# CVMI-Lab/DODA

Hardware: AMD Instinct MI355X
Metric: active-voxels/sec fwd+bwd SparseConv U-Net, ScanNet 2cm (higher is better)
Workload: dtype bf16; 1 GPU; cfgs/scannet SparseConv U-Net training step (voxel pooling + fwd + CE + bwd + SGD), 2 cm voxels, 4 scenes/GPU x ~150000 active voxels, random-init weights; global_batch=4, voxels_per_gpu=601279, points_per_gpu=781042, parallelism=dp1, n_classes=20, grad_sync=deferred multi-layer wgrad + bucketed all-reduce, collectives=none (single process), prefetch_gate=off, grad_exchange=no process group

## Files before the change

doda_amd/csrc/spconv_wlds.hip:

```cpp
#include "common.hpp"
#include "spconv_common.hpp"

namespace {

constexpr int WK = 27, WCH = 48, WNB = 3;
constexpr int W_SLOTS = 96;
constexpr int W_LDS_BYTES = WK * WNB * W_SLOTS * 16;

template <int S, bool STATS>
__device__ __forceinline__ void wlds_epilogue(f32x4 (&acc)[S], const u32x2 (&pre_res)[S], const u32x2 (&pre_bnx)[S], int row0,
                                              int i, int g, int wid, int nb, int n_out, __amdgpu_buffer_rsrc_t rs_y,
                                              const void *__restrict__ res, const EpiArgs &ep, int part, f32x4 (*sred)[2][4],
                                              const float (*bnv)[WCH]) {
    const unsigned col = (unsigned)(nb * 16 + 4 * g);
    f32x4 st1 = {0.f, 0.f, 0.f, 0.f}, st2 = {0.f, 0.f, 0.f, 0.f};
    auto unpack = [](const u32x2 &v) {
        return (f32x4){__uint_as_float(v[0] << 16), __uint_as_float(v[0] & 0xffff0000u),
                       __uint_as_float(v[1] << 16), __uint_as_float(v[1] & 0xffff0000u)};
    };
#pragma unroll
    for (int s = 0; s < S; ++s) {
        const unsigned t = (unsigned)(row0 + s * 16 + i);
        const unsigned voff = t < (unsigned)n_out ? (t * (ep.y_ld ? ep.y_ld : (unsigned)WCH) + col) * 2u : OOB;
        f32x4 a = acc[s];
        if (res) a += unpack(pre_res[s]);
        u32x2 packed_out;
        packed_out[0] = (unsigned)f2bf(a[0]) | ((unsigned)f2bf(a[1]) << 16);
        packed_out[1] = (unsigned)f2bf(a[2]) | ((unsigned)f2bf(a[3]) << 16);
        if constexpr (STATS) {
            f32x4 v = unpack(packed_out);
            if (ep.bn_x) {
                const f32x4 xr = unpack(pre_bnx[s]);
                const f32x4 mu = *reinterpret_cast<const f32x4 *>(&bnv[0][col]);
                const f32x4 is = *reinterpret_cast<const f32x4 *>(&bnv[1][col]);
                const f32x4 xh = (xr - mu) * is;
                if (ep.bn_relu) {
                    const f32x4 ga = *reinterpret_cast<const f32x4 *>(&bnv[2][col]);
                    const f32x4 be = *reinterpret_cast<const f32x4 *>(&bnv[3][col]);
                    const f32x4 yv = xh * ga + be;
#pragma unroll
                    for (int q = 0; q < 4; ++q) v[q] = yv[q] > 0.f ? v[q] : 0.f;
                }
                st1 += v;
                st2 += v * xh;
            } else {
                st1 += v;
                st2 += v * v;
            }
        }
        __builtin_amdgcn_raw_buffer_store_b64(packed_out, rs_y, voff, 0, 0);
    }
    if constexpr (STATS) {
#pragma unroll
        for (int q = 0; q < 4; ++q) { st1[q] = row_sum16(st1[q]); st2[q] = row_sum16(st2[q]); }
        if (i == 15) { sred[wid][0][g] = st1; sred[wid][1][g] = st2; }
        doda_sync();
        if (wid == 0 && i == 15) {
            f32x4 a1 = sred[0][0][g], a2 = sred[0][1][g];
#pragma unroll
            for (int w = 1; w < 8; ++w) { a1 += sred[w][0][g]; a2 += sred[w][1][g]; }
            stats_emit(ep, (long long)part, WCH, col, a1, a2);
        }
        doda_sync();
    }
}

template <bool STATS>
__global__ __launch_bounds__(512) void conv_wlds48(const unsigned short *__restrict__ x, unsigned x_bytes,
                                                   const u32x4 *__restrict__ wp, const int32_t *__restrict__ tbl,
                                                   unsigned tbl_bytes, int ld, int n_out, void *__restrict__ y,
                                                   unsigned y_bytes, const void *__restrict__ res, const EpiArgs ep) {
    constexpr int S = 2, RW = 16 * S, TM = 8 * RW;
    extern __shared__ __attribute__((aligned(16))) unsigned char wl_raw[];
    u32x4 *wl = reinterpret_cast<u32x4 *>(wl_raw);
    __shared__ f32x4 sred[STATS ? 8 : 1][2][4];
    __shared__ __attribute__((aligned(16))) float bnv[4][WCH];

    const int tid = threadIdx.x, lane = tid & 63, wid = __builtin_amdgcn_readfirstlane(tid >> 6);
    const int i = lane & 15, g = lane >> 4;
    const __amdgpu_buffer_rsrc_t rs_x = __builtin_amdgcn_make_buffer_rsrc((void *)x, 0, x_bytes, 0x00020000);
    const __amdgpu_buffer_rsrc_t rs_t = __builtin_amdgcn_make_buffer_rsrc((void *)tbl, 0, tbl_bytes, 0x00020000);
    const __amdgpu_buffer_rsrc_t rs_y = __builtin_amdgcn_make_buffer_rsrc((void *)y, 0, y_bytes, 0x00020000);

    if constexpr (STATS) {
        if (ep.bn_x && tid < 4 * WCH) {
            const int v = tid / WCH, c = tid - v * WCH;
            const float *src = v == 0 ? ep.bn_mean : v == 1 ? ep.bn_invstd : v == 2 ? ep.bn_gamma : ep.bn_beta;
            bnv[v][c] = src ? src[c] : 0.f;
        }
    }
    const int n_tiles = (n_out + TM - 1) / TM;
    unsigned off[WK][S];
    auto load_table = [&](int tile) {
        const int row0 = tile * TM + wid * RW;
#pragma unroll
        for (int o = 0; o < WK; ++o)
#pragma unroll
            for (int s = 0; s < S; ++s) {
                const int t = row0 + s * 16 + i;
                const unsigned voff = t < n_out ? ((unsigned)o * (unsigned)ld + (unsigned)t) * 4u : OOB;
                off[o][s] = __builtin_amdgcn_raw_buffer_load_b32(rs_t, voff, 0, 0);
            }
    };
    {
        constexpr int NCP = (WK * WNB * W_SLOTS + 511) / 512;
        u32x4 tmp[NCP];
#pragma unroll
        for (int k = 0; k < NCP; ++k) {
            const int e = k * 512 + tid, ec = e < WK * WNB * W_SLOTS ? e : 0;
            const int slot = ec % W_SLOTS, onb = ec / W_SLOTS, nb = onb % WNB, o = onb / WNB;
            const int src = slot < 64 ? ((o * 2 + 0) * WNB + nb) * 64 + slot : ((o * 2 + 1) * WNB + nb) * 64 + (slot - 64);
            tmp[k] = wp[src];
        }
        load_table((int)blockIdx.x);
#pragma unroll
        for (int k = 0; k < NCP; ++k) {
            const int e = k * 512 + tid;
            if (e < WK * WNB * W_SLOTS) wl[e] = tmp[k];
        }
    }
    doda_sync();

    for (int tile = blockIdx.x; tile < n_tiles; tile += gridDim.x) {
        const int row0 = tile * TM + wid * RW;
        u32x2 pre_res[WNB][S], pre_bnx[WNB][S];
        {
            const unsigned rl = ep.res_ld ? ep.res_ld : (unsigned)WCH, bl = ep.bnx_ld ? ep.bnx_ld : (unsigned)WCH;
            const unsigned dense_bytes = (unsigned)n_out * (unsigned)WCH * 2u;
            const __amdgpu_buffer_rsrc_t rs_r = __builtin_amdgcn_make_buffer_rsrc(
                (void *)res, 0, ep.res_ld ? ((unsigned)(n_out - 1) * rl + (unsigned)WCH) * 2u : dense_bytes, 0x00020000);
            const __amdgpu_buffer_rsrc_t rs_b = __builtin_amdgcn_make_buffer_rsrc(
                (void *)ep.bn_x, 0, ep.bnx_ld ? ((unsigned)(n_out - 1) * bl + (unsigned)WCH) * 2u : dense_bytes, 0x00020000);
#pragma unroll
            for (int nb = 0; nb < WNB; ++nb)
#pragma unroll
                for (int s = 0; s < S; ++s) {
                    const unsigned t = (unsigned)(row0 + s * 16 + i);
                    const unsigned cc = (unsigned)(nb * 16 + 4 * g);
                    const unsigned voff = t < (unsigned)n_out ? (t * rl + cc) * 2u : OOB;
                    const unsigned voff_b = t < (unsigned)n_out ? (t * bl + cc) * 2u : OOB;
                    pre_res[nb][s] = __builtin_amdgcn_raw_buffer_load_b64(rs_r, res ? voff : OOB, 0, 0);
                    if constexpr (STATS) pre_bnx[nb][s] = __builtin_amdgcn_raw_buffer_load_b64(rs_b, ep.bn_x ? voff_b : OOB, 0, 0);
                    else pre_bnx[nb][s] = (u32x2){0u, 0u};
                }
        }
        if (tile != (int)blockIdx.x) load_table(tile);
#pragma unroll
        for (int o = 0; o < WK; ++o)
#pragma unroll
            for (int s = 0; s < S; ++s) {
                const int t = row0 + s * 16 + i;
                off[o][s] = (t < n_out && (int)off[o][s] >= 0) ? off[o][s] * (unsigned)(WCH * 2) : OOB;
            }

        f32x4 acc[WNB][S];
#pragma unroll
        for (int nb = 0; nb < WNB; ++nb)
#pragma unroll
            for (int s = 0; s < S; ++s) acc[nb][s] = (f32x4){0.f, 0.f, 0.f, 0.f};

        auto gather = [&](int u, u32x4 (&xa)[S]) {
            const int o = u >> 1, c = u & 1;
#pragma unroll
            for (int s = 0; s < S; ++s) {
                const unsigned base = off[o][s];
                const unsigned voff = (c == 0 || g < 2) && base != OOB ? base + (unsigned)(c * 64 + g * 16) : OOB;
                xa[s] = __builtin_amdgcn_raw_buffer_load_b128(rs_x, voff, 0, 0);
            }
        };
        constexpr int NUNIT = 2 * WK;
        constexpr int PD = 4;
        u32x4 xa[PD + 1][S];
#pragma unroll
        for (int u = 0; u < PD; ++u) gather(u, xa[u]);
#pragma unroll
        for (int u = 0; u < NUNIT; ++u) {
            if (u + PD < NUNIT) gather(u + PD, xa[(u + PD) % (PD + 1)]);
            const int o = u >> 1, c = u & 1;
            u32x4 wf[WNB];
#pragma unroll
            for (int nb = 0; nb < WNB; ++nb) {
                const u32x4 *frag = wl + (o * WNB + nb) * W_SLOTS;
                wf[nb] = c == 0 ? frag[lane] : (g < 2 ? frag[64 + lane] : (u32x4){0u, 0u, 0u, 0u});
            }
            __builtin_amdgcn_sched_barrier(0);
#pragma unroll
            for (int nb = 0; nb < WNB; ++nb)
#pragma unroll
                for (int s = 0; s < S; ++s) mma_bf16_k32(acc[nb][s], wf[nb], xa[u % (PD + 1)][s]);
            __builtin_amdgcn_sched_barrier(0);
        }
#pragma unroll
        for (int nb = 0; nb < WNB; ++nb)
            wlds_epilogue<S, STATS>(acc[nb], pre_res[nb], pre_bnx[nb], row0, i, g, wid, nb, n_out, rs_y, res, ep, tile, sred, bnv);
    }
}

}

int doda_wlds::launch(const GatherRoute &r, const GatherOperands &a, hipStream_t s) {
    static bool attr_done = false;
    if (!attr_done) {
        if (hipFuncSetAttribute((const void *)conv_wlds48<true>, hipFuncAttributeMaxDynamicSharedMemorySize, W_LDS_BYTES) != hipSuccess ||
            hipFuncSetAttribute((const void *)conv_wlds48<false>, hipFuncAttributeMaxDynamicSharedMemorySize, W_LDS_BYTES) != hipSuccess)
            return DODA_ERR_LAUNCH;
        attr_done = true;
    }
    with_bool(r.stats, [&](auto ST) {
        hipLaunchKernelGGL((conv_wlds48<decltype(ST)::value>), dim3(r.grid), dim3(r.block), W_LDS_BYTES, s, (const unsigned short *)a.x, r.x_bytes,
                           (const u32x4 *)a.wp, a.tbl, r.tbl_bytes, a.ld, a.n_out, a.y, r.y_bytes, a.res, a.ep);
    });
    return doda_check_launch();
}
```

Measured before the change: 138.3 million voxels/s.

## Deepen gather prefetch, double-buffer LDS weight fragments, batch epilogue barriers

Restructures the LDS-weight 48-channel gather conv kernel. The input gather prefetch depth goes from 4 to 8, and weight fragments for the next unit are read from LDS one step ahead into a double buffer. The first tile's table load and gathers now overlap the weight staging. BN stats reductions for all three column blocks share one barrier pair per tile instead of three, and the trailing barrier is skipped on the last tile. LDS addressing is split into two base pointers so offsets fit 16-bit immediates. The cost is many more live registers (xa grows to 9xS b128, plus wf x2), which risks lower occupancy or spills.

```diff
diff --git a/doda_amd/csrc/spconv_wlds.hip b/doda_amd/csrc/spconv_wlds.hip
--- a/doda_amd/csrc/spconv_wlds.hip
+++ b/doda_amd/csrc/spconv_wlds.hip
@@ -6,62 +6,73 @@
 constexpr int WK = 27, WCH = 48, WNB = 3;
 constexpr int W_SLOTS = 96;
 constexpr int W_LDS_BYTES = WK * WNB * W_SLOTS * 16;
+constexpr int W_HI_SLOT = 42;
+static_assert(((W_HI_SLOT - 1) * W_SLOTS + 64) * 16 < 65536 && ((WK * WNB - W_HI_SLOT - 1) * W_SLOTS + 64) * 16 < 65536, "LDS offsets are 16 bits");
+constexpr int W_PD = 8;
 
 template <int S, bool STATS>
-__device__ __forceinline__ void wlds_epilogue(f32x4 (&acc)[S], const u32x2 (&pre_res)[S], const u32x2 (&pre_bnx)[S], int row0,
-                                              int i, int g, int wid, int nb, int n_out, __amdgpu_buffer_rsrc_t rs_y,
-                                              const void *__restrict__ res, const EpiArgs &ep, int part, f32x4 (*sred)[2][4],
-                                              const float (*bnv)[WCH]) {
-    const unsigned col = (unsigned)(nb * 16 + 4 * g);
-    f32x4 st1 = {0.f, 0.f, 0.f, 0.f}, st2 = {0.f, 0.f, 0.f, 0.f};
+__device__ __forceinline__ void wlds_epilogue(f32x4 (&acc)[WNB][S], const u32x2 (&pre_res)[WNB][S], const u32x2 (&pre_bnx)[WNB][S],
+                                              int row0, int i, int g, int wid, int n_out, __amdgpu_buffer_rsrc_t rs_y,
+                                              const void *__restrict__ res, const EpiArgs &ep, int part, bool more,
+                                              f32x4 (*sred)[WNB][2][4], const float (*bnv)[WCH]) {
     auto unpack = [](const u32x2 &v) {
         return (f32x4){__uint_as_float(v[0] << 16), __uint_as_float(v[0] & 0xffff0000u),
                        __uint_as_float(v[1] << 16), __uint_as_float(v[1] & 0xffff0000u)};
     };
 #pragma unroll
-    for (int s = 0; s < S; ++s) {
-        const unsigned t = (unsigned)(row0 + s * 16 + i);
-        const unsigned voff = t < (unsigned)n_out ? (t * (ep.y_ld ? ep.y_ld : (unsigned)WCH) + col) * 2u : OOB;
-        f32x4 a = acc[s];
-        if (res) a += unpack(pre_res[s]);
-        u32x2 packed_out;
-        packed_out[0] = (unsigned)f2bf(a[0]) | ((unsigned)f2bf(a[1]) << 16);
-        packed_out[1] = (unsigned)f2bf(a[2]) | ((unsigned)f2bf(a[3]) << 16);
+    for (int nb = 0; nb < WNB; ++nb) {
+        const unsigned col = (unsigned)(nb * 16 + 4 * g);
+        f32x4 st1 = {0.f, 0.f, 0.f, 0.f}, st2 = {0.f, 0.f, 0.f, 0.f};
+#pragma unroll
+        for (int s = 0; s < S; ++s) {
+            const unsigned t = (unsigned)(row0 + s * 16 + i);
+            const unsigned voff = t < (unsigned)n_out ? (t * (ep.y_ld ? ep.y_ld : (unsigned)WCH) + col) * 2u : OOB;
+            f32x4 a = acc[nb][s];
+            if (res) a += unpack(pre_res[nb][s]);
+            u32x2 packed_out;
+            packed_out[0] = (unsigned)f2bf(a[0]) | ((unsigned)f2bf(a[1]) << 16);
+            packed_out[1] = (unsigned)f2bf(a[2]) | ((unsigned)f2bf(a[3]) << 16);
+            if constexpr (STATS) {
+                f32x4 v = unpack(packed_out);
+                if (ep.bn_x) {
+                    const f32x4 xr = unpack(pre_bnx[nb][s]);
+                    const f32x4 mu = *reinterpret_cast<const f32x4 *>(&bnv[0][col]);
+                    const f32x4 is = *reinterpret_cast<const f32x4 *>(&bnv[1][col]);
+                    const f32x4 xh = (xr - mu) * is;
+                    if (ep.bn_relu) {
+                        const f32x4 ga = *reinterpret_cast<const f32x4 *>(&bnv[2][col]);
+                        const f32x4 be = *reinterpret_cast<const f32x4 *>(&bnv[3][col]);
+                        const f32x4 yv = xh * ga + be;
+#pragma unroll
+                        for (int q = 0; q < 4; ++q) v[q] = yv[q] > 0.f ? v[q] : 0.f;
+                    }
+                    st1 += v;
+                    st2 += v * xh;
+                } else {
+                    st1 += v;
+                    st2 += v * v;
+                }
+            }
+            __builtin_amdgcn_raw_buffer_store_b64(packed_out, rs_y, voff, 0, 0);
+        }
         if constexpr (STATS) {
-            f32x4 v = unpack(packed_out);
-            if (ep.bn_x) {
-                const f32x4 xr = unpack(pre_bnx[s]);
-                const f32x4 mu = *reinterpret_cast<const f32x4 *>(&bnv[0][col]);
-                const f32x4 is = *reinterpret_cast<const f32x4 *>(&bnv[1][col]);
-                const f32x4 xh = (xr - mu) * is;
-                if (ep.bn_relu) {
-                    const f32x4 ga = *reinterpret_cast<const f32x4 *>(&bnv[2][col]);
-                    const f32x4 be = *reinterpret_cast<const f32x4 *>(&bnv[3][col]);
-                    const f32x4 yv = xh * ga + be;
-#pragma unroll
-                    for (int q = 0; q < 4; ++q) v[q] = yv[q] > 0.f ? v[q] : 0.f;
-                }
-                st1 += v;
-                st2 += v * xh;
-            } else {
-                st1 += v;
-                st2 += v * v;
-            }
-        }
-        __builtin_amdgcn_raw_buffer_store_b64(packed_out, rs_y, voff, 0, 0);
+#pragma unroll
+            for (int q = 0; q < 4; ++q) { st1[q] = row_sum16(st1[q]); st2[q] = row_sum16(st2[q]); }
+            if (i == 15) { sred[wid][nb][0][g] = st1; sred[wid][nb][1][g] = st2; }
+        }
     }
     if constexpr (STATS) {
-#pragma unroll
-        for (int q = 0; q < 4; ++q) { st1[q] = row_sum16(st1[q]); st2[q] = row_sum16(st2[q]); }
-        if (i == 15) { sred[wid][0][g] = st1; sred[wid][1][g] = st2; }
         doda_sync();
         if (wid == 0 && i == 15) {
-            f32x4 a1 = sred[0][0][g], a2 = sred[0][1][g];
-#pragma unroll
-            for (int w = 1; w < 8; ++w) { a1 += sred[w][0][g]; a2 += sred[w][1][g]; }
-            stats_emit(ep, (long long)part, WCH, col, a1, a2);
-        }
-        doda_sync();
+#pragma nounroll
+            for (int nb = 0; nb < WNB; ++nb) {
+                f32x4 a1 = sred[0][nb][0][g], a2 = sred[0][nb][1][g];
+#pragma unroll
+                for (int w = 1; w < 8; ++w) { a1 += sred[w][nb][0][g]; a2 += sred[w][nb][1][g]; }
+                stats_emit(ep, (long long)part, WCH, nb * 16 + 4 * g, a1, a2);
+            }
+        }
+        if (more) doda_sync();
     }
 }
 
@@ -71,22 +82,32 @@
                                                    unsigned tbl_bytes, int ld, int n_out, void *__restrict__ y,
                                                    unsigned y_bytes, const void *__restrict__ res, const EpiArgs ep) {
     constexpr int S = 2, RW = 16 * S, TM = 8 * RW;
+    constexpr int PD = W_PD;
     extern __shared__ __attribute__((aligned(16))) unsigned char wl_raw[];
     u32x4 *wl = reinterpret_cast<u32x4 *>(wl_raw);
-    __shared__ f32x4 sred[STATS ? 8 : 1][2][4];
+    __shared__ f32x4 sred[STATS ? 8 : 1][WNB][2][4];
     __shared__ __attribute__((aligned(16))) float bnv[4][WCH];
+    __shared__ unsigned wl_split;
 
     const int tid = threadIdx.x, lane = tid & 63, wid = __builtin_amdgcn_readfirstlane(tid >> 6);
     const int i = lane & 15, g = lane >> 4;
     const __amdgpu_buffer_rsrc_t rs_x = __builtin_amdgcn_make_buffer_rsrc((void *)x, 0, x_bytes, 0x00020000);
     const __amdgpu_buffer_rsrc_t rs_t = __builtin_amdgcn_make_buffer_rsrc((void *)tbl, 0, tbl_bytes, 0x00020000);
     const __amdgpu_buffer_rsrc_t rs_y = __builtin_amdgcn_make_buffer_rsrc((void *)y, 0, y_bytes, 0x00020000);
-
+    const __amdgpu_buffer_rsrc_t rs_w = __builtin_amdgcn_make_buffer_rsrc((void *)wp, 0, WK * 2 * WNB * 64 * 16, 0x00020000);
+    const unsigned rl = ep.res_ld ? ep.res_ld : (unsigned)WCH, bl = ep.bnx_ld ? ep.bnx_ld : (unsigned)WCH;
+    const unsigned dense_bytes = (unsigned)n_out * (unsigned)WCH * 2u;
+    const __amdgpu_buffer_rsrc_t rs_r = __builtin_amdgcn_make_buffer_rsrc(
+        (void *)res, 0, ep.res_ld ? ((unsigned)(n_out - 1) * rl + (unsigned)WCH) * 2u : dense_bytes, 0x00020000);
+    const __amdgpu_buffer_rsrc_t rs_b = __builtin_amdgcn_make_buffer_rsrc(
+        (void *)ep.bn_x, 0, ep.bnx_ld ? ((unsigned)(n_out - 1) * bl + (unsigned)WCH) * 2u : dense_bytes, 0x00020000);
+
+    float bn_val = 0.f;
     if constexpr (STATS) {
         if (ep.bn_x && tid < 4 * WCH) {
             const int v = tid / WCH, c = tid - v * WCH;
             const float *src = v == 0 ? ep.bn_mean : v == 1 ? ep.bn_invstd : v == 2 ? ep.bn_gamma : ep.bn_beta;
-            bnv[v][c] = src ? src[c] : 0.f;
+            if (src) bn_val = src[c];
         }
     }
     const int n_tiles = (n_out + TM - 1) / TM;
@@ -102,6 +123,45 @@
                 off[o][s] = __builtin_amdgcn_raw_buffer_load_b32(rs_t, voff, 0, 0);
             }
     };
+    auto gather = [&](int u, u32x4 (&xa)[S]) {
+        const int o = u >> 1, c = u & 1;
+#pragma unroll
+        for (int s = 0; s < S; ++s) {
+            const unsigned voff = (c == 0 || g < 2 ? off[o][s] : OOB) + (unsigned)(c * 64);
+            xa[s] = __builtin_amdgcn_raw_buffer_load_b128(rs_x, voff, 0, 0);
+        }
+    };
+    constexpr int NUNIT = 2 * WK;
+    u32x4 xa[PD + 1][S];
+    u32x2 pre_res[WNB][S], pre_bnx[WNB][S];
+    auto tile_head = [&](int tile) {
+        const int row0 = tile * TM + wid * RW;
+#pragma unroll
+        for (int o = 0; o < WK; ++o)
+#pragma unroll
+            for (int s = 0; s < S; ++s) {
+                const int t = row0 + s * 16 + i;
+                off[o][s] = (t < n_out && (int)off[o][s] >= 0) ? off[o][s] * (unsigned)(WCH * 2) + (unsigned)(g * 16) : OOB;
+            }
+#pragma unroll
+        for (int u = 0; u < PD; ++u) gather(u, xa[u]);
+    };
+    auto tile_operands = [&](int tile) {
+        const int row0 = tile * TM + wid * RW;
+#pragma unroll
+        for (int nb = 0; nb < WNB; ++nb)
+#pragma unroll
+            for (int s = 0; s < S; ++s) {
+                const unsigned t = (unsigned)(row0 + s * 16 + i);
+                const unsigned cc = (unsigned)(nb * 16 + 4 * g);
+                const unsigned voff = t < (unsigned)n_out ? (t * rl + cc) * 2u : OOB;
+                const unsigned voff_b = t < (unsigned)n_out ? (t * bl + cc) * 2u : OOB;
+                pre_res[nb][s] = __builtin_amdgcn_raw_buffer_load_b64(rs_r, res ? voff : OOB, 0, 0);
+                if constexpr (STATS) pre_bnx[nb][s] = __builtin_amdgcn_raw_buffer_load_b64(rs_b, ep.bn_x ? voff_b : OOB, 0, 0);
+                else pre_bnx[nb][s] = (u32x2){0u, 0u};
+            }
+    };
+    load_table((int)blockIdx.x);
     {
         constexpr int NCP = (WK * WNB * W_SLOTS + 511) / 512;
         u32x4 tmp[NCP];
@@ -110,89 +170,61 @@
             const int e = k * 512 + tid, ec = e < WK * WNB * W_SLOTS ? e : 0;
             const int slot = ec % W_SLOTS, onb = ec / W_SLOTS, nb = onb % WNB, o = onb / WNB;
             const int src = slot < 64 ? ((o * 2 + 0) * WNB + nb) * 64 + slot : ((o * 2 + 1) * WNB + nb) * 64 + (slot - 64);
-            tmp[k] = wp[src];
-        }
-        load_table((int)blockIdx.x);
+            tmp[k] = __builtin_amdgcn_raw_buffer_load_b128(rs_w, (unsigned)src * 16u, 0, 0);
+        }
+        tile_head((int)blockIdx.x);
+        __builtin_amdgcn_sched_barrier(0);
 #pragma unroll
         for (int k = 0; k < NCP; ++k) {
             const int e = k * 512 + tid;
             if (e < WK * WNB * W_SLOTS) wl[e] = tmp[k];
         }
-    }
+        tile_operands((int)blockIdx.x);
+    }
+    if constexpr (STATS) {
+        if (ep.bn_x && tid < 4 * WCH) (&bnv[0][0])[tid] = bn_val;
+    }
+    if (tid == 0) wl_split = (unsigned)W_HI_SLOT * W_SLOTS;
     doda_sync();
+    const u32x4 *wl_lo = wl + lane, *wl_hi = wl_lo + __builtin_amdgcn_readfirstlane(*(volatile unsigned *)&wl_split);
 
     for (int tile = blockIdx.x; tile < n_tiles; tile += gridDim.x) {
         const int row0 = tile * TM + wid * RW;
-        u32x2 pre_res[WNB][S], pre_bnx[WNB][S];
-        {
-            const unsigned rl = ep.res_ld ? ep.res_ld : (unsigned)WCH, bl = ep.bnx_ld ? ep.bnx_ld : (unsigned)WCH;
-            const unsigned dense_bytes = (unsigned)n_out * (unsigned)WCH * 2u;
-            const __amdgpu_buffer_rsrc_t rs_r = __builtin_amdgcn_make_buffer_rsrc(
-                (void *)res, 0, ep.res_ld ? ((unsigned)(n_out - 1) * rl + (unsigned)WCH) * 2u : dense_bytes, 0x00020000);
-            const __amdgpu_buffer_rsrc_t rs_b = __builtin_amdgcn_make_buffer_rsrc(
-                (void *)ep.bn_x, 0, ep.bnx_ld ? ((unsigned)(n_out - 1) * bl + (unsigned)WCH) * 2u : dense_bytes, 0x00020000);
-#pragma unroll
-            for (int nb = 0; nb < WNB; ++nb)
-#pragma unroll
-                for (int s = 0; s < S; ++s) {
-                    const unsigned t = (unsigned)(row0 + s * 16 + i);
-                    const unsigned cc = (unsigned)(nb * 16 + 4 * g);
-                    const unsigned voff = t < (unsigned)n_out ? (t * rl + cc) * 2u : OOB;
-                    const unsigned voff_b = t < (unsigned)n_out ? (t * bl + cc) * 2u : OOB;
-                    pre_res[nb][s] = __builtin_amdgcn_raw_buffer_load_b64(rs_r, res ? voff : OOB, 0, 0);
-                    if constexpr (STATS) pre_bnx[nb][s] = __builtin_amdgcn_raw_buffer_load_b64(rs_b, ep.bn_x ? voff_b : OOB, 0, 0);
-                    else pre_bnx[nb][s] = (u32x2){0u, 0u};
-                }
-        }
-        if (tile != (int)blockIdx.x) load_table(tile);
-#pragma unroll
-        for (int o = 0; o < WK; ++o)
-#pragma unroll
-            for (int s = 0; s < S; ++s) {
-                const int t = row0 + s * 16 + i;
-                off[o][s] = (t < n_out && (int)off[o][s] >= 0) ? off[o][s] * (unsigned)(WCH * 2) : OOB;
-            }
-
+        if (tile != (int)blockIdx.x) {
+            load_table(tile);
+            tile_head(tile);
+            tile_operands(tile);
+        }
         f32x4 acc[WNB][S];
 #pragma unroll
         for (int nb = 0; nb < WNB; ++nb)
 #pragma unroll
             for (int s = 0; s < S; ++s) acc[nb][s] = (f32x4){0.f, 0.f, 0.f, 0.f};
 
-        auto gather = [&](int u, u32x4 (&xa)[S]) {
+        auto fragments = [&](int u, u32x4 (&wf)[WNB]) {
             const int o = u >> 1, c = u & 1;
 #pragma unroll
-            for (int s = 0; s < S; ++s) {
-                const unsigned base = off[o][s];
-                const unsigned voff = (c == 0 || g < 2) && base != OOB ? base + (unsigned)(c * 64 + g * 16) : OOB;
-                xa[s] = __builtin_amdgcn_raw_buffer_load_b128(rs_x, voff, 0, 0);
+            for (int nb = 0; nb < WNB; ++nb) {
+                const int slot = o * WNB + nb;
+                const u32x4 *frag = slot < W_HI_SLOT ? wl_lo + slot * W_SLOTS : wl_hi + (slot - W_HI_SLOT) * W_SLOTS;
+                wf[nb] = c == 0 ? frag[0] : (g < 2 ? frag[64] : (u32x4){0u, 0u, 0u, 0u});
             }
         };
-        constexpr int NUNIT = 2 * WK;
-        constexpr int PD = 4;
-        u32x4 xa[PD + 1][S];
-#pragma unroll
-        for (int u = 0; u < PD; ++u) gather(u, xa[u]);
+        u32x4 wf[2][WNB];
+        fragments(0, wf[0]);
 #pragma unroll
         for (int u = 0; u < NUNIT; ++u) {
             if (u + PD < NUNIT) gather(u + PD, xa[(u + PD) % (PD + 1)]);
-            const int o = u >> 1, c = u & 1;
-            u32x4 wf[WNB];
-#pragma unroll
-            for (int nb = 0; nb < WNB; ++nb) {
-                const u32x4 *frag = wl + (o * WNB + nb) * W_SLOTS;
-                wf[nb] = c == 0 ? frag[lane] : (g < 2 ? frag[64 + lane] : (u32x4){0u, 0u, 0u, 0u});
-            }
+            if (u + 1 < NUNIT) fragments(u + 1, wf[(u + 1) & 1]);
             __builtin_amdgcn_sched_barrier(0);
 #pragma unroll
             for (int nb = 0; nb < WNB; ++nb)
 #pragma unroll
-                for (int s = 0; s < S; ++s) mma_bf16_k32(acc[nb][s], wf[nb], xa[u % (PD + 1)][s]);
+                for (int s = 0; s < S; ++s) mma_bf16_k32(acc[nb][s], wf[u & 1][nb], xa[u % (PD + 1)][s]);
             __builtin_amdgcn_sched_barrier(0);
         }
-#pragma unroll
-        for (int nb = 0; nb < WNB; ++nb)
-            wlds_epilogue<S, STATS>(acc[nb], pre_res[nb], pre_bnx[nb], row0, i, g, wid, nb, n_out, rs_y, res, ep, tile, sred, bnv);
+        wlds_epilogue<S, STATS>(acc, pre_res, pre_bnx, row0, i, g, wid, n_out, rs_y, res, ep, tile, tile + (int)gridDim.x < n_tiles,
+                                sred, bnv);
     }
 }
 
```

Measured after the change: 138.7 million voxels/s, median of 3. About the same (+0.3%).
